# MingXiangL/SPE

Measured on AMD Instinct MI355X. Metric: images/sec (whole node) at 3x800x1333 bs=2/GPU, higher is better.
Workload: dtype bf16/fp16 operands, fp32 accumulate; 1 GPU; TSCAM_cait_S24 (C=384, depth 24, 8 heads) + 0-layer encoder + 6-layer conditional-DETR decoder x2 stages, 100 queries, COCO heads (91), 2x3x800x1333 per GPU (N=4150 tokens), fwd + SetCriterion + SetCriterionRefine + bwd + grad all-reduce + clip + AdamW; global_batch=2, parallelism=dp1

## Files before the change

### spe_amd/csrc/gemm_nt2.hip

```cpp
#include <cstdlib>
#include "common.h"
#include "gemm16_epilogue.h"
#include "gemm_nt_select.h"
#include "gemm_tiles.h"

template <int CPR>
__device__ __forceinline__ int nt2_swz(int r) {
    if constexpr (CPR == 8) return r & 7;
    else return (0x78 >> (2 * ((r >> 2) & 3))) & 3;
}

template <int BM, int BN, int BK, int NST, bool SPLIT, bool EX, bool F16>
__global__ __launch_bounds__(256, 2) void gemm_nt2_kernel(Gemm16Args p) {
    extern __shared__ __attribute__((aligned(16))) unsigned short smem16[];
    constexpr int NFM = BM / 32, NFN = BN / 32, WM = BM / 2, WN = BN / 2;
    constexpr int CPR = BK / 8;
    constexpr int RPP = 64 / CPR;
    constexpr int PA = BM / RPP, PB = BN / RPP;
    constexpr int NP = (PA + PB) * (SPLIT ? 2 : 1), PW = NP / 4;
    constexpr int STE = NP * 512;
    static_assert(NP % 4 == 0 && BM % 32 == 0 && BN % 32 == 0 && (BK == 32 || BK == 64) && NST >= 2, "tile geometry");

    const int tiles_m = (p.M + BM - 1) / BM, tiles_n = (p.N + BN - 1) / BN;
    int tm, tn;
    if (!tile_decode(p.xcd_bind, tiles_m, tiles_n, tm, tn)) return;
    const int m0 = tm * BM, n0 = tn * BN;
    if (p.stagger > 0 && (blockIdx.x >> 8) == 1) {
        for (int i = 0; i < p.stagger; ++i) __builtin_amdgcn_s_sleep(127);
    }
#if defined(SPE_ABLATE) && defined(SPE_ABL_NOLOOP)
    const int nt = 1;
#else
    const int nt = p.K / BK;
#endif

    const int lane = threadIdx.x & 63, w = threadIdx.x >> 6;
    const int ws = __builtin_amdgcn_readfirstlane(w);
    const int wm = w >> 1, wn = w & 1;
    const int fr = lane & 15, fc = lane >> 4;
    const unsigned lds0 = __builtin_amdgcn_readfirstlane((unsigned)(uintptr_t)(__attribute__((address_space(3))) unsigned short*)smem16);

    f32x4_t acc[NFM][NFN];
#pragma unroll
    for (int i = 0; i < NFM; ++i)
#pragma unroll
        for (int j = 0; j < NFN; ++j) acc[i][j] = (f32x4_t){0.f, 0.f, 0.f, 0.f};

    const int pr = lane / CPR, pc = lane % CPR;
    auto issue = [&](int t, int slot) {
        const int tc = min(t, nt - 1);
        const long k0 = (long)tc * BK;
#pragma unroll
        for (int i = 0; i < PW; ++i) {
            const int piece = i * 4 + ws;
            constexpr int HALF = PA + PB;
            const bool lo = SPLIT && (piece >= HALF);
            const int ph = lo ? piece - HALF : piece;
            const bool isA = ph < PA;
            const int r = (isA ? ph : ph - PA) * RPP + pr;
            const int gc = pc ^ nt2_swz<CPR>(r);
            const unsigned short* base = isA ? (lo ? p.Alo : p.A) : (lo ? p.Blo : p.B);
            const unsigned short* src = isA ? base + (long)min(m0 + r, p.M - 1) * p.lda + k0 + gc * 8
                                            : base + (long)min(n0 + r, p.N - 1) * p.ldb + k0 + gc * 8;
            glds16(src, lds0 + (unsigned)((slot * STE + piece * 512) * 2));
        }
    };
#pragma unroll
    for (int st = 0; st < NST - 1; ++st) issue(st, st);
    for (int t = 0; t < nt; ++t) {
        asm volatile("s_waitcnt vmcnt(%0)" :: "n"((NST - 2) * PW) : "memory");
        __builtin_amdgcn_s_barrier();
        asm volatile("" ::: "memory");
        issue(t + NST - 1, (t + NST - 1) % NST);
        const unsigned short* sA_ = smem16 + (t % NST) * STE;
        const unsigned short* sB_ = sA_ + PA * 512;
        const unsigned short* sAl = sA_ + (PA + PB) * 512;
        const unsigned short* sBl = sAl + PA * 512;
#pragma unroll
        for (int ks = 0; ks < BK / 32; ++ks) {
            const int kc = ks * 4 + fc;
            bf16x8_t a[NFM], b[NFN], al[SPLIT ? NFM : 1], bl[SPLIT ? NFN : 1];
#pragma unroll
            for (int i = 0; i < NFM; ++i) {
                const int row = wm * WM + i * 16 + fr;
                const int off = row * BK + ((kc ^ nt2_swz<CPR>(row)) * 8);
                a[i] = __builtin_bit_cast(bf16x8_t, *reinterpret_cast<const u16x8_t*>(sA_ + off));
                if constexpr (SPLIT) al[i] = __builtin_bit_cast(bf16x8_t, *reinterpret_cast<const u16x8_t*>(sAl + off));
            }
#pragma unroll
            for (int j = 0; j < NFN; ++j) {
                const int row = wn * WN + j * 16 + fr;
                const int off = row * BK + ((kc ^ nt2_swz<CPR>(row)) * 8);
                b[j] = __builtin_bit_cast(bf16x8_t, *reinterpret_cast<const u16x8_t*>(sB_ + off));
                if constexpr (SPLIT) bl[j] = __builtin_bit_cast(bf16x8_t, *reinterpret_cast<const u16x8_t*>(sBl + off));
            }
            if constexpr (SPLIT) {
#pragma unroll
                for (int i = 0; i < NFM; ++i)
#pragma unroll
                    for (int j = 0; j < NFN; ++j) acc[i][j] = __builtin_amdgcn_mfma_f32_16x16x32_bf16(bl[j], a[i], acc[i][j], 0, 0, 0);
#pragma unroll
                for (int i = 0; i < NFM; ++i)
#pragma unroll
                    for (int j = 0; j < NFN; ++j) acc[i][j] = __builtin_amdgcn_mfma_f32_16x16x32_bf16(b[j], al[i], acc[i][j], 0, 0, 0);
            }
#pragma unroll
            for (int i = 0; i < NFM; ++i)
#pragma unroll
                for (int j = 0; j < NFN; ++j) {
                    if constexpr (F16) {
                        typedef _Float16 nt2_h8_t __attribute__((ext_vector_type(8)));
                        acc[i][j] = __builtin_amdgcn_mfma_f32_16x16x32_f16(__builtin_bit_cast(nt2_h8_t, b[j]), __builtin_bit_cast(nt2_h8_t, a[i]), acc[i][j], 0, 0, 0);
                    } else acc[i][j] = __builtin_amdgcn_mfma_f32_16x16x32_bf16(b[j], a[i], acc[i][j], 0, 0, 0);
                }
        }
    }
    asm volatile("s_waitcnt vmcnt(0)" ::: "memory");
    __syncthreads();
#if defined(SPE_ABLATE) && defined(SPE_ABL_NOSTORE)
#pragma unroll
    for (int i = 0; i < NFM; ++i)
#pragma unroll
        for (int j = 0; j < NFN; ++j) asm volatile("" :: "v"(acc[i][j]));
    return;
#endif
    if constexpr (EX) gemm16_epilogue_ex<BM, BN, SPLIT || F16, false>(p, acc, smem16, m0, n0);
    else if (F16 && (p.h16 & 2) && (p.N & 7) == 0 && (p.ldc & 7) == 0) gemm16_epilogue_h16<BM, BN>(p, acc, smem16, m0, n0);
    else gemm16_epilogue_plain<BM, BN>(p, acc, p.C, m0, n0);
}

template <int BM, int BN, int BK, int NST, bool SPLIT, bool EX, bool F16>
int launch_nt2(const Gemm16Args& p, hipStream_t stream) {
    constexpr int ring = NST * ((BM + BN) / (64 / (BK / 8))) * (SPLIT ? 2 : 1) * 1024;
    constexpr int epi = EX ? BM * (BN + 8) * 2 * ((SPLIT || F16) ? 2 : 1) : 0;
    constexpr int smem = ring > epi ? ring : epi;
    static bool attr_set = false;
    if (!attr_set) {
        hipError_t e = hipFuncSetAttribute(reinterpret_cast<const void*>(&gemm_nt2_kernel<BM, BN, BK, NST, SPLIT, EX, F16>),
                                           hipFuncAttributeMaxDynamicSharedMemorySize, smem);
        if (e != hipSuccess) return (int)e;
        attr_set = true;
    }
    const int tiles_m = (p.M + BM - 1) / BM, tiles_n = (p.N + BN - 1) / BN;
    const TileOrder order = tile_order(p.M, p.N, tiles_m, tiles_n);
    Gemm16Args q = p;
    q.xcd_bind = order.xcd_bind;
    q.stagger = 0;
    const DetDeferSeg sg[1] = {{q.colsum, q.N}};
    float* region = (EX && q.colsum) ? det_defer_try(tiles_n, tiles_m, BN, 1, sg, stream) : nullptr;
    if (region) q.ws.defer = region;
    hipLaunchKernelGGL((gemm_nt2_kernel<BM, BN, BK, NST, SPLIT, EX, F16>), dim3(order.grid), dim3(256), smem, stream, q);
    if (region) det_defer_commit(region, tiles_n, tiles_m, BN, 1, sg, 1);
    SPE_CHECK_LAUNCH();
    return 0;
}
#define NT2_INSTANTIATE(BM, BN, BK, NST, SPLIT, EX, F16) template int launch_nt2<BM, BN, BK, NST, SPLIT, EX, F16>(const Gemm16Args&, hipStream_t);
NT2_INSTANCES(NT2_INSTANTIATE)
#undef NT2_INSTANTIATE
```

### spe_amd/csrc/gemm_tiles.h

```cpp
#pragma once

struct TileOrder {
    int xcd_bind;
    int grid;
};

static inline TileOrder tile_order(int M, int N, int tiles_m, int tiles_n) {
    TileOrder o{0, tiles_m * tiles_n};
    if (M >= N && tiles_m >= 16) o.xcd_bind = 1;
    else if (N > M && tiles_n >= 16) o.xcd_bind = 2;
    else if (tiles_m >= 16) o.xcd_bind = 1;
    else if (tiles_n >= 16) o.xcd_bind = 2;
    if (o.xcd_bind == 1) o.grid = 8 * ((tiles_m + 7) / 8) * tiles_n;
    if (o.xcd_bind == 2) o.grid = 8 * ((tiles_n + 7) / 8) * tiles_m;
    return o;
}

__device__ __forceinline__ bool tile_decode(int xcd_bind, int tiles_m, int tiles_n, int& tm, int& tn) {
    if (xcd_bind == 0) { tm = blockIdx.x % tiles_m; tn = blockIdx.x / tiles_m; }
    else {
        const int no = (xcd_bind == 1) ? tiles_n : tiles_m;
        const int xcd = blockIdx.x & 7, idx = blockIdx.x >> 3;
        const int tb = xcd + 8 * (idx / no), to = idx % no;
        tm = (xcd_bind == 1) ? tb : to; tn = (xcd_bind == 1) ? to : tb;
        if (tm >= tiles_m || tn >= tiles_n) return false;
    }
    return true;
}

__device__ __forceinline__ void glds16(const void* gsrc, unsigned lds_dst) {
    unsigned keep;
    asm volatile("s_mov_b32 %0, m0\n\ts_mov_b32 m0, %2\n\ts_nop 0\n\tglobal_load_lds_dwordx4 %1, off\n\ts_mov_b32 m0, %0"
                 : "=&s"(keep) : "v"(gsrc), "s"(lds_dst) : "memory");
}
```

Baseline: 41.80 images/sec.

## Restructure nt2 GEMM mainloop with SGPR-based loads, fragment prefetch, peeled tail

Precomputes per-lane 32-bit global offsets and scalar base pointers so each LDS-direct load uses the saddr+voffset form, with M0 set by a single scalar add instead of being saved and restored each time. The mainloop now double-buffers LDS fragments across k-substeps, with sched barriers so fragment reads overlap the MFMAs. The last NST-1 iterations are peeled out so they issue no redundant clamped loads. A host check rejects leading dimensions whose offsets would overflow 32 bits, and there is a possible SGPR/m0 clobber risk since m0 is no longer restored.

```diff
diff --git a/spe_amd/csrc/gemm_nt2.hip b/spe_amd/csrc/gemm_nt2.hip
--- a/spe_amd/csrc/gemm_nt2.hip
+++ b/spe_amd/csrc/gemm_nt2.hip
@@ -4,10 +4,11 @@
 #include "gemm_nt_select.h"
 #include "gemm_tiles.h"
 
-template <int CPR>
-__device__ __forceinline__ int nt2_swz(int r) {
-    if constexpr (CPR == 8) return r & 7;
-    else return (0x78 >> (2 * ((r >> 2) & 3))) & 3;
+template <int I, int PW, int STEP>
+__device__ __forceinline__ void nt2_issue(const unsigned char* (&sb)[PW], const unsigned (&vo)[PW], unsigned lds_stage) {
+    nt2_glds16<I * 4096>(sb[I], vo[I], lds_stage);
+    sb[I] += STEP;
+    if constexpr (I + 1 < PW) nt2_issue<I + 1, PW, STEP>(sb, vo, lds_stage);
 }
 
 template <int BM, int BN, int BK, int NST, bool SPLIT, bool EX, bool F16>
@@ -46,76 +47,93 @@
 #pragma unroll
         for (int j = 0; j < NFN; ++j) acc[i][j] = (f32x4_t){0.f, 0.f, 0.f, 0.f};
 
-    const int pr = lane / CPR, pc = lane % CPR;
-    auto issue = [&](int t, int slot) {
-        const int tc = min(t, nt - 1);
-        const long k0 = (long)tc * BK;
+    const unsigned char* sb[PW];
+    unsigned vo[PW];
 #pragma unroll
-        for (int i = 0; i < PW; ++i) {
-            const int piece = i * 4 + ws;
-            constexpr int HALF = PA + PB;
-            const bool lo = SPLIT && (piece >= HALF);
-            const int ph = lo ? piece - HALF : piece;
-            const bool isA = ph < PA;
-            const int r = (isA ? ph : ph - PA) * RPP + pr;
-            const int gc = pc ^ nt2_swz<CPR>(r);
-            const unsigned short* base = isA ? (lo ? p.Alo : p.A) : (lo ? p.Blo : p.B);
-            const unsigned short* src = isA ? base + (long)min(m0 + r, p.M - 1) * p.lda + k0 + gc * 8
-                                            : base + (long)min(n0 + r, p.N - 1) * p.ldb + k0 + gc * 8;
-            glds16(src, lds0 + (unsigned)((slot * STE + piece * 512) * 2));
+    for (int i = 0; i < PW; ++i) {
+        const Nt2Piece q = nt2_piece(BM, BN, BK, SPLIT, i * 4 + ws);
+        const bool isA = (q.arr & 1) == 0;
+        const unsigned short* base = q.arr == 0 ? p.A : q.arr == 1 ? p.B : q.arr == 2 ? p.Alo : p.Blo;
+        sb[i] = reinterpret_cast<const unsigned char*>(base + (isA ? (long)m0 * p.lda : (long)n0 * p.ldb));
+        vo[i] = nt2_lane_off(BK, q.row0, lane, isA ? m0 : n0, isA ? p.M : p.N, isA ? p.lda : p.ldb);
+    }
+    const unsigned ldw = lds0 + nt2_piece_lds(NP, 0, ws);
+
+    struct Frag { bf16x8_t a[NFM], b[NFN], al[SPLIT ? NFM : 1], bl[SPLIT ? NFN : 1]; };
+    auto ldfrag = [&](Frag& f, const unsigned short* sA_, int ks) {
+        const unsigned short* sB_ = sA_ + PA * 512;
+        const unsigned short* sAl = sA_ + (PA + PB) * 512;
+        const unsigned short* sBl = sAl + PA * 512;
+        const int kc = ks * 4 + fc;
+#pragma unroll
+        for (int i = 0; i < NFM; ++i) {
+            const int row = wm * WM + i * 16 + fr;
+            const int off = row * BK + ((kc ^ nt2_swz(CPR, row)) * 8);
+            f.a[i] = __builtin_bit_cast(bf16x8_t, *reinterpret_cast<const u16x8_t*>(sA_ + off));
+            if constexpr (SPLIT) f.al[i] = __builtin_bit_cast(bf16x8_t, *reinterpret_cast<const u16x8_t*>(sAl + off));
+        }
+#pragma unroll
+        for (int j = 0; j < NFN; ++j) {
+            const int row = wn * WN + j * 16 + fr;
+            const int off = row * BK + ((kc ^ nt2_swz(CPR, row)) * 8);
+            f.b[j] = __builtin_bit_cast(bf16x8_t, *reinterpret_cast<const u16x8_t*>(sB_ + off));
+            if constexpr (SPLIT) f.bl[j] = __builtin_bit_cast(bf16x8_t, *reinterpret_cast<const u16x8_t*>(sBl + off));
         }
     };
+    auto mma = [&](const Frag& f) {
+        if constexpr (SPLIT) {
 #pragma unroll
-    for (int st = 0; st < NST - 1; ++st) issue(st, st);
-    for (int t = 0; t < nt; ++t) {
+            for (int i = 0; i < NFM; ++i)
+#pragma unroll
+                for (int j = 0; j < NFN; ++j) acc[i][j] = __builtin_amdgcn_mfma_f32_16x16x32_bf16(f.bl[j], f.a[i], acc[i][j], 0, 0, 0);
+#pragma unroll
+            for (int i = 0; i < NFM; ++i)
+#pragma unroll
+                for (int j = 0; j < NFN; ++j) acc[i][j] = __builtin_amdgcn_mfma_f32_16x16x32_bf16(f.b[j], f.al[i], acc[i][j], 0, 0, 0);
+        }
+#pragma unroll
+        for (int i = 0; i < NFM; ++i)
+#pragma unroll
+            for (int j = 0; j < NFN; ++j) {
+                if constexpr (F16) {
+                    typedef _Float16 nt2_h8_t __attribute__((ext_vector_type(8)));
+                    acc[i][j] = __builtin_amdgcn_mfma_f32_16x16x32_f16(__builtin_bit_cast(nt2_h8_t, f.b[j]), __builtin_bit_cast(nt2_h8_t, f.a[i]), acc[i][j], 0, 0, 0);
+                } else acc[i][j] = __builtin_amdgcn_mfma_f32_16x16x32_bf16(f.b[j], f.a[i], acc[i][j], 0, 0, 0);
+            }
+    };
+    auto stage = [&](int t, bool refill) {
+        constexpr bool FRAG_FIRST = BM == 64;
+        const unsigned short* sA_ = smem16 + (t % NST) * STE;
+        Frag f[BK / 32];
+        if constexpr (FRAG_FIRST) ldfrag(f[0], sA_, 0);
+        if (refill) nt2_issue<0, PW, BK * 2>(sb, vo, ldw + (unsigned)((t + NST - 1) % NST) * (STE * 2));
+        if constexpr (!FRAG_FIRST) ldfrag(f[0], sA_, 0);
+#pragma unroll
+        for (int ks = 0; ks < BK / 32; ++ks) {
+            if (ks + 1 < BK / 32) {
+                ldfrag(f[ks + 1], sA_, ks + 1);
+                __builtin_amdgcn_sched_barrier(0);
+            }
+            mma(f[ks]);
+        }
+    };
+
+#pragma unroll
+    for (int st = 0; st < NST - 1; ++st) nt2_issue<0, PW, BK * 2>(sb, vo, ldw + (unsigned)st * (STE * 2));
+    __builtin_amdgcn_s_waitcnt(0xC07F);
+    for (int t = 0; t < nt - (NST - 1); ++t) {
         asm volatile("s_waitcnt vmcnt(%0)" :: "n"((NST - 2) * PW) : "memory");
         __builtin_amdgcn_s_barrier();
         asm volatile("" ::: "memory");
-        issue(t + NST - 1, (t + NST - 1) % NST);
-        const unsigned short* sA_ = smem16 + (t % NST) * STE;
-        const unsigned short* sB_ = sA_ + PA * 512;
-        const unsigned short* sAl = sA_ + (PA + PB) * 512;
-        const unsigned short* sBl = sAl + PA * 512;
+        stage(t, true);
+    }
 #pragma unroll
-        for (int ks = 0; ks < BK / 32; ++ks) {
-            const int kc = ks * 4 + fc;
-            bf16x8_t a[NFM], b[NFN], al[SPLIT ? NFM : 1], bl[SPLIT ? NFN : 1];
-#pragma unroll
-            for (int i = 0; i < NFM; ++i) {
-                const int row = wm * WM + i * 16 + fr;
-                const int off = row * BK + ((kc ^ nt2_swz<CPR>(row)) * 8);
-                a[i] = __builtin_bit_cast(bf16x8_t, *reinterpret_cast<const u16x8_t*>(sA_ + off));
-                if constexpr (SPLIT) al[i] = __builtin_bit_cast(bf16x8_t, *reinterpret_cast<const u16x8_t*>(sAl + off));
-            }
-#pragma unroll
-            for (int j = 0; j < NFN; ++j) {
-                const int row = wn * WN + j * 16 + fr;
-                const int off = row * BK + ((kc ^ nt2_swz<CPR>(row)) * 8);
-                b[j] = __builtin_bit_cast(bf16x8_t, *reinterpret_cast<const u16x8_t*>(sB_ + off));
-                if constexpr (SPLIT) bl[j] = __builtin_bit_cast(bf16x8_t, *reinterpret_cast<const u16x8_t*>(sBl + off));
-            }
-            if constexpr (SPLIT) {
-#pragma unroll
-                for (int i = 0; i < NFM; ++i)
-#pragma unroll
-                    for (int j = 0; j < NFN; ++j) acc[i][j] = __builtin_amdgcn_mfma_f32_16x16x32_bf16(bl[j], a[i], acc[i][j], 0, 0, 0);
-#pragma unroll
-                for (int i = 0; i < NFM; ++i)
-#pragma unroll
-                    for (int j = 0; j < NFN; ++j) acc[i][j] = __builtin_amdgcn_mfma_f32_16x16x32_bf16(b[j], al[i], acc[i][j], 0, 0, 0);
-            }
-#pragma unroll
-            for (int i = 0; i < NFM; ++i)
-#pragma unroll
-                for (int j = 0; j < NFN; ++j) {
-                    if constexpr (F16) {
-                        typedef _Float16 nt2_h8_t __attribute__((ext_vector_type(8)));
-                        acc[i][j] = __builtin_amdgcn_mfma_f32_16x16x32_f16(__builtin_bit_cast(nt2_h8_t, b[j]), __builtin_bit_cast(nt2_h8_t, a[i]), acc[i][j], 0, 0, 0);
-                    } else acc[i][j] = __builtin_amdgcn_mfma_f32_16x16x32_bf16(b[j], a[i], acc[i][j], 0, 0, 0);
-                }
-        }
+    for (int j = 0; j < NST - 1; ++j) {
+        asm volatile("s_waitcnt vmcnt(0)" ::: "memory");
+        __builtin_amdgcn_s_barrier();
+        asm volatile("" ::: "memory");
+        stage(nt - (NST - 1) + j, false);
     }
-    asm volatile("s_waitcnt vmcnt(0)" ::: "memory");
     __syncthreads();
 #if defined(SPE_ABLATE) && defined(SPE_ABL_NOSTORE)
 #pragma unroll
@@ -134,6 +152,7 @@
     constexpr int ring = NST * ((BM + BN) / (64 / (BK / 8))) * (SPLIT ? 2 : 1) * 1024;
     constexpr int epi = EX ? BM * (BN + 8) * 2 * ((SPLIT || F16) ? 2 : 1) : 0;
     constexpr int smem = ring > epi ? ring : epi;
+    if (!nt2_offsets_fit(p.lda, p.ldb)) return -2;
     static bool attr_set = false;
     if (!attr_set) {
         hipError_t e = hipFuncSetAttribute(reinterpret_cast<const void*>(&gemm_nt2_kernel<BM, BN, BK, NST, SPLIT, EX, F16>),
diff --git a/spe_amd/csrc/gemm_tiles.h b/spe_amd/csrc/gemm_tiles.h
--- a/spe_amd/csrc/gemm_tiles.h
+++ b/spe_amd/csrc/gemm_tiles.h
@@ -1,4 +1,10 @@
 #pragma once
+
+#if defined(__HIPCC__)
+#define GT_HD __host__ __device__ __forceinline__
+#else
+#define GT_HD inline
+#endif
 
 struct TileOrder {
     int xcd_bind;
@@ -16,6 +22,7 @@
     return o;
 }
 
+#if defined(__HIPCC__)
 __device__ __forceinline__ bool tile_decode(int xcd_bind, int tiles_m, int tiles_n, int& tm, int& tn) {
     if (xcd_bind == 0) { tm = blockIdx.x % tiles_m; tn = blockIdx.x / tiles_m; }
     else {
@@ -27,9 +34,34 @@
     }
     return true;
 }
+#endif
 
-__device__ __forceinline__ void glds16(const void* gsrc, unsigned lds_dst) {
-    unsigned keep;
-    asm volatile("s_mov_b32 %0, m0\n\ts_mov_b32 m0, %2\n\ts_nop 0\n\tglobal_load_lds_dwordx4 %1, off\n\ts_mov_b32 m0, %0"
-                 : "=&s"(keep) : "v"(gsrc), "s"(lds_dst) : "memory");
+
+GT_HD int nt2_swz(int CPR, int r) { return CPR == 8 ? (r & 7) : ((0x78 >> (2 * ((r >> 2) & 3))) & 3); }
+
+struct Nt2Piece {
+    int arr;
+    int row0;
+};
+GT_HD Nt2Piece nt2_piece(int BM, int BN, int BK, bool SPLIT, int piece) {
+    const int RPP = 512 / BK, PA = BM / RPP, PB = BN / RPP;
+    const bool lo = SPLIT && piece >= PA + PB;
+    const int ph = lo ? piece - (PA + PB) : piece;
+    return Nt2Piece{(ph < PA ? 0 : 1) + (lo ? 2 : 0), (ph < PA ? ph : ph - PA) * RPP};
 }
+GT_HD unsigned nt2_piece_lds(int NP, int slot, int piece) { return (unsigned)(slot * NP + piece) * 1024u; }
+
+GT_HD unsigned nt2_lane_off(int BK, int row0, int lane, int t0, int rows, long ld) {
+    const int CPR = BK / 8, r = row0 + lane / CPR, pc = lane % CPR;
+    const int rc = (t0 + r < rows ? t0 + r : rows - 1) - t0;
+    return (unsigned)((long)rc * ld * 2 + (pc ^ nt2_swz(CPR, r)) * 16);
+}
+GT_HD bool nt2_offsets_fit(long lda, long ldb) { return 160 * (lda > ldb ? lda : ldb) * 2 <= 0x7fffffffL; }
+
+#if defined(__HIPCC__)
+template <int LDS_OFF>
+__device__ __forceinline__ void nt2_glds16(const void* sbase, unsigned voff, unsigned lds_base) {
+    asm volatile("s_add_u32 m0, %2, %3\n\ts_nop 0\n\tglobal_load_lds_dwordx4 %0, %1"
+                 :: "v"(voff), "s"(sbase), "s"(lds_base), "n"(LDS_OFF) : "memory", "scc");
+}
+#endif
```

Result: no change. 42.12 images/sec (median of 6 runs) (+0.8%).
